# AdalineL/Multi-Modal-GNN

Hardware: AMD Instinct MI355X
Metric: has_lab edges/s, one full training step (new 20 % supervision mask + fwd + weighted-MAE loss + bwd + Adam) of predict_lab_values on the full hetero-graph; message passing over every edge, the two edge heads evaluated on the supervised pairs (the only predictions the loss reads, train.py:366-370) (higher is better)
Workload: dtype f32; 1 GPU; eICU-shape synthetic hetero-graph x100 per GPU, 128-d, 2 SAGE layers x 6 relations, dropout 0.2, supervision mask (20%) redrawn inside every step; patients_per_gpu=183400, has_lab_edges_total=6148400, train_pairs_rank0=4303880, hidden_dim=128, parallelism=single GPU, ranks=1, launch=hipGraph replay

## Files before the change

include/mmgnn.h:

```cpp
#ifndef MMGNN_H
#define MMGNN_H

#include <stddef.h>
#include <stdint.h>

#ifdef __cplusplus
extern "C" {
#endif

#define MMG_OK 0
#define MMG_E_ARG (-1)
#define MMG_E_LAUNCH (-2)
#define MMG_E_WS (-3)

#define MMG_MAX_REL 4

int mmg_version(void);
const char* mmg_last_error(void);

int mmg_stream_create(void** stream_out);
int mmg_stream_destroy(void* stream);

size_t mmg_csr_build_ws_bytes(int64_t n_edges, int64_t n_rows);
int mmg_csr_build(const int64_t* edge_index, int64_t n_edges, int64_t n_rows, int sort_row,
// ... 296 lines not shown
  float drop_p;
  uint64_t seed; uint32_t site; int64_t row_offset; const uint64_t* seed_ptr;
} mmg_small_bn_t;
typedef struct {
  const float* G; const float* Y; float* dY;
  const float* scale; const float* shift; const float* mean; const float* rstd;
  float* dbeta; float* dgamma;
  int64_t M;
  int training;
  int act;
  float drop_p;
  uint64_t seed; uint32_t site; int64_t row_offset; const uint64_t* seed_ptr;
} mmg_small_bn_bwd_t;
int mmg_small_bn_act_group(const mmg_small_bn_t* probs, int n_probs, int N, float momentum, float eps, void* stream);
int mmg_small_bn_bwd_group(const mmg_small_bn_bwd_t* probs, int n_probs, int N, void* stream);

#define MMG_ADAM_MAX_TENSORS 96
#define MMG_SUM_MAX_JOBS 8
int mmg_adam_step(float* p, float* m, float* v, const float* const* grads, const int32_t* offsets, int n_tensors,
                  float lr, float beta1, float beta2, float eps, float weight_decay, float* step, uint32_t* ticket,
                  void* stream);
int mmg_adam_step_dev(float* p, float* m, float* v, const float* const* grads, const int32_t* offsets, int n_tensors,
                      const float* hyper, float* step, uint32_t* ticket, void* stream);
typedef struct {
  float* dst;
  const float* src[4];
  int n_src;
  int len;
  int cols;
  int ld_dst;
  int ld_src[4];
} mmg_sum_job_t;
int mmg_vec_sums(const mmg_sum_job_t* jobs, int n_jobs, void* stream);
#define MMG_COUNTERS_MAX 32
int mmg_counters_add(int64_t* const* counters, const int64_t* incs, int n, void* stream);
int mmg_seed_advance(uint64_t* state , void* stream);
int mmg_fill_zero(void* ptr, size_t bytes, void* stream);

size_t mmg_seg_reduce_ws_bytes(int64_t n, int n_seg);
int mmg_seg_moments(const float* pred, const float* target, const int64_t* seg, int64_t n, int n_seg,
                    double* moments, void* ws, size_t ws_bytes, void* stream);
int mmg_seg_metrics(const float* pred, const float* target, const int64_t* seg, int64_t n, int n_seg,
                    const double* moments, float n_sigma, float* pred_out, double* sums, void* ws, size_t ws_bytes,
                    void* stream);

size_t mmg_knn_impute_ws_bytes(int64_t n_rows, int n_cols, int64_t n_out, int n_neighbors);
int mmg_knn_impute(const float* X, int64_t n_rows, int n_cols, int64_t ld_x, const int32_t* rows, int64_t n_out,
                   int n_neighbors, int weights , float* out, int64_t ld_out, void* ws,
                   size_t ws_bytes, void* stream);

#define MMG_OS_MAX_RANKS 8
size_t mmg_order_stats_ws_bytes(int64_t n);
int mmg_order_stats(const float* a, const float* b, int64_t n, const int64_t* ranks, int n_ranks, float* out,
                    int64_t* nan_count, void* ws, size_t ws_bytes, void* stream);

typedef struct {
  int32_t lo, hi;
  float g;
} mmg_percentile_t;
// ... 124 lines not shown
```

multi-modal-gnn_amd/csrc/optim.hip:

```cpp
#include "common.h"

namespace {

struct AdamTable {
  const float* grad[MMG_ADAM_MAX_TENSORS];
  int32_t off[MMG_ADAM_MAX_TENSORS + 1];
  int n;
};

__global__ __launch_bounds__(256) void k_adam(AdamTable tb, float* __restrict__ p, float* __restrict__ m,
                                              float* __restrict__ v, float lr, float b1, float b2, float eps, float wd,
                                              const float* __restrict__ hyper, const float* __restrict__ step) {
  if (hyper) { lr = hyper[0]; b1 = hyper[1]; b2 = hyper[2]; eps = hyper[3]; wd = hyper[4]; }
  __shared__ float s_bc[3];
  __shared__ int s_off[MMG_ADAM_MAX_TENSORS + 1];
  __shared__ const float* s_grad[MMG_ADAM_MAX_TENSORS];
  for (int i = threadIdx.x; i <= tb.n; i += 256) s_off[i] = tb.off[i];
  for (int i = threadIdx.x; i < tb.n; i += 256) s_grad[i] = tb.grad[i];
  if (threadIdx.x == 0) {
    const float t0 = *step + 1.f;
    s_bc[0] = t0; s_bc[1] = 1.f - powf(b1, t0); s_bc[2] = sqrtf(1.f - powf(b2, t0));
  }
  __syncthreads();
  const float bc1 = s_bc[1], bc2s = s_bc[2];
// ... 40 lines not shown
  const int j = blockIdx.y;
  const int n = jb.len[j], cols = jb.cols[j];
  for (int i = blockIdx.x * 256 + threadIdx.x; i < n; i += gridDim.x * 256) {
    const int r = i / cols, c = i - r * cols;
    float s = jb.src[j][0][(size_t)r * jb.ld_src[j][0] + c];
    for (int q = 1; q < jb.n_src[j]; ++q) s += jb.src[j][q][(size_t)r * jb.ld_src[j][q] + c];
    jb.dst[j][(size_t)r * jb.ld_dst[j] + c] = s;
  }
}

struct CounterTable { int64_t* p[MMG_COUNTERS_MAX]; int64_t inc[MMG_COUNTERS_MAX]; int n; };
__global__ void k_counters_add(CounterTable tb) {
  const int i = threadIdx.x;
  if (i < tb.n) *tb.p[i] += tb.inc[i];
}

__global__ void k_seed_advance(uint64_t* state) {
  uint64_t z = (state[1] += 0x9E3779B97F4A7C15ull);
  z = (z ^ (z >> 30)) * 0xBF58476D1CE4E5B9ull;
  z = (z ^ (z >> 27)) * 0x94D049BB133111EBull;
  state[0] = (z ^ (z >> 31)) >> 2;
}

}

static int adam_launch(float* p, float* m, float* v, const float* const* grads, const int32_t* offsets, int n_tensors,
                       float lr, float beta1, float beta2, float eps, float weight_decay, const float* hyper, float* step,
                       uint32_t* ticket, void* stream) {
  MMG_CHECK_ARG(p && m && v && grads && offsets && step && ticket, "adam_step: null buffer");
  MMG_CHECK_ARG(n_tensors >= 1, "adam_step: no tensors");
  hipStream_t st = (hipStream_t)stream;
  for (int t0 = 0; t0 < n_tensors; t0 += MMG_ADAM_MAX_TENSORS) {
    AdamTable tb;
    const int n = n_tensors - t0 < MMG_ADAM_MAX_TENSORS ? n_tensors - t0 : MMG_ADAM_MAX_TENSORS;
    tb.n = n;
    for (int i = 0; i < n; ++i) { tb.grad[i] = grads[t0 + i]; tb.off[i] = offsets[t0 + i]; }
    tb.off[n] = offsets[t0 + n];
    MMG_CHECK_ARG(tb.off[n] >= tb.off[0], "adam_step: offsets must ascend");
    const int total = tb.off[n] - tb.off[0];
    int nb = (total + 256 * 2 - 1) / (256 * 2);
    if (nb < 1) nb = 1;
    if (nb > 2048) nb = 2048;
    hipLaunchKernelGGL(k_adam, dim3(nb), dim3(256), 0, st, tb, p, m, v, lr, beta1, beta2, eps, weight_decay, hyper, step);
  }
  hipLaunchKernelGGL(k_adam_bump, dim3(1), dim3(1), 0, st, step);
  MMG_CHECK_LAUNCH("adam_step");
  return MMG_OK;
}

extern "C" int mmg_adam_step(float* p, float* m, float* v, const float* const* grads, const int32_t* offsets, int n_tensors,
                             float lr, float beta1, float beta2, float eps, float weight_decay, float* step,
                             uint32_t* ticket, void* stream) {
  return adam_launch(p, m, v, grads, offsets, n_tensors, lr, beta1, beta2, eps, weight_decay, nullptr, step, ticket, stream);
}

extern "C" int mmg_adam_step_dev(float* p, float* m, float* v, const float* const* grads, const int32_t* offsets,
                                 int n_tensors, const float* hyper, float* step, uint32_t* ticket, void* stream) {
  MMG_CHECK_ARG(hyper, "adam_step_dev: null hyper-parameter buffer");
  return adam_launch(p, m, v, grads, offsets, n_tensors, 0.f, 0.f, 0.f, 0.f, 0.f, hyper, step, ticket, stream);
}

extern "C" int mmg_vec_sums(const mmg_sum_job_t* jobs, int n_jobs, void* stream) {
  MMG_CHECK_ARG(jobs && n_jobs >= 1 && n_jobs <= MMG_SUM_MAX_JOBS, "vec_sums: 1..%d jobs", MMG_SUM_MAX_JOBS);
  SumJobs jb;
  jb.n = n_jobs;
  int maxlen = 0;
  for (int j = 0; j < n_jobs; ++j) {
    MMG_CHECK_ARG(jobs[j].dst && jobs[j].n_src >= 1 && jobs[j].n_src <= 4 && jobs[j].len >= 0, "vec_sums: bad job %d", j);
    jb.dst[j] = jobs[j].dst; jb.n_src[j] = jobs[j].n_src; jb.len[j] = jobs[j].len;
    const int cols = jobs[j].cols;
    MMG_CHECK_ARG(cols >= 0 && (cols == 0 || jobs[j].len % cols == 0), "vec_sums: job %d: len is not a multiple of cols", j);
    jb.cols[j] = cols > 0 ? cols : (jobs[j].len > 0 ? jobs[j].len : 1);
    jb.ld_dst[j] = cols > 0 ? jobs[j].ld_dst : 0;
    MMG_CHECK_ARG(cols == 0 || jobs[j].ld_dst >= cols, "vec_sums: job %d: ld_dst < cols", j);
    for (int q = 0; q < 4; ++q) {
      jb.src[j][q] = q < jobs[j].n_src ? jobs[j].src[q] : nullptr;
      jb.ld_src[j][q] = cols > 0 ? jobs[j].ld_src[q] : 0;
      MMG_CHECK_ARG(cols == 0 || q >= jobs[j].n_src || jobs[j].ld_src[q] >= cols, "vec_sums: job %d: ld_src < cols", j);
    }
    for (int q = 0; q < jobs[j].n_src; ++q) MMG_CHECK_ARG(jobs[j].src[q], "vec_sums: job %d has a null source", j);
    if (jobs[j].len > maxlen) maxlen = jobs[j].len;
    for (int i = 0; i < j; ++i) MMG_CHECK_ARG(jobs[i].dst != jobs[j].dst, "vec_sums: jobs %d and %d share a destination", i, j);
// ... 8 lines not shown

extern "C" int mmg_counters_add(int64_t* const* counters, const int64_t* incs, int n, void* stream) {
  MMG_CHECK_ARG(n >= 0 && n <= MMG_COUNTERS_MAX, "counters_add: 0..%d counters", MMG_COUNTERS_MAX);
  if (n == 0) return MMG_OK;
  MMG_CHECK_ARG(counters && incs, "counters_add: null table");
  CounterTable tb;
  tb.n = n;
  for (int i = 0; i < n; ++i) {
    MMG_CHECK_ARG(counters[i], "counters_add: counter %d is null", i);
    tb.p[i] = counters[i]; tb.inc[i] = incs[i];
  }
  hipLaunchKernelGGL(k_counters_add, dim3(1), dim3(64), 0, (hipStream_t)stream, tb);
  MMG_CHECK_LAUNCH("counters_add");
  return MMG_OK;
}

extern "C" int mmg_seed_advance(uint64_t* state, void* stream) {
  MMG_CHECK_ARG(state, "seed_advance: null state");
  hipLaunchKernelGGL(k_seed_advance, dim3(1), dim3(1), 0, (hipStream_t)stream, state);
  MMG_CHECK_LAUNCH("seed_advance");
  return MMG_OK;
}

extern "C" int mmg_fill_zero(void* ptr, size_t bytes, void* stream) {
  if (bytes == 0) return MMG_OK;
  MMG_CHECK_ARG(ptr, "fill_zero: null buffer");
  MMG_CHECK_HIP(mmg_zero_async(ptr, bytes, (hipStream_t)stream), "fill_zero");
  return MMG_OK;
}
```

multi-modal-gnn_amd/model.py:

```python
from __future__ import annotations

import logging
from dataclasses import dataclass, field
from typing import Dict, List, NamedTuple, Optional, Tuple

import torch
import torch.nn as nn
import torch.nn.functional as F

from . import _lib, ops
from .data import GraphPlan, LAB_EDGE, ROW_TYPE, RelCSR, build_plan
from .ops import Pro

EdgeType = Tuple[str, str, str]
SITE_CONV = 16
SITE_H1 = 64
SITE_TYPES_PER_LAYER = 8


def check_dropout_sites(num_layers: int, n_node_types: int):
    if n_node_types > SITE_TYPES_PER_LAYER:
        raise ValueError(f"{n_node_types} node types: the dropout sites of a conv layer hold {SITE_TYPES_PER_LAYER}")
    if SITE_CONV + SITE_TYPES_PER_LAYER * num_layers > SITE_H1:
        raise ValueError(f"num_layers={num_layers}: the dropout sites of the conv layers would run into the pair heads' "
# ... 16 lines not shown

def set_next_bn(sites):
    global NEXT_BN_SITES
    sites = frozenset(sites)
    if not sites <= {"heads", "conv", "enc2", "enc1"}:
        raise ValueError(f"unknown next-BatchNorm site(s): {sorted(sites - {'heads', 'conv', 'enc2', 'enc1'})}")
    NEXT_BN_SITES = sites


FUSED_WGRAD = True


def set_fused_wgrad(on: bool):
    global FUSED_WGRAD
    FUSED_WGRAD = bool(on)


DUAL_ENC = True


def set_dual_enc(on: bool):
    global DUAL_ENC
    DUAL_ENC = bool(on)


FUSED_HEAD_WGRAD = True


def set_fused_head_wgrad(on: bool):
    global FUSED_HEAD_WGRAD
    FUSED_HEAD_WGRAD = bool(on)


def _mangle(et: EdgeType) -> str:
    return "<" + "___".join(et) + ">"


class HeadLists(NamedTuple):
    sel_low: torch.Tensor
    sel_high: torch.Tensor
    counts: torch.Tensor
    n_low: int
    n_high: int
    low_rows: torch.Tensor
    pi_low: torch.Tensor
    deg_low: torch.Tensor
# ... 290 lines not shown
    src: dict
    head: ops.Head
    w1a: torch.Tensor
    w1b: torch.Tensor
    xP: object
    save: Optional[tuple]


class _StepFn(torch.autograd.Function):
    @staticmethod
    def forward(ctx, run, mode, n_out, *params):
        ctx.run = run
        outs = run.run_forward(mode)
        ctx.mark_non_differentiable(*[o for o in outs if not o.is_floating_point()])
        return tuple(outs)

    @staticmethod
    def backward(ctx, *gouts):
        grads = ctx.run.run_backward(gouts)
        return (None, None, None) + tuple(grads)


class _Run:
    def __init__(self, model: HeteroRGCN, data):
        self.m = model
        self.dev = next(model.parameters()).device
        if self.dev.type != "cuda":
            raise ops._lib.MmgError("HeteroRGCN runs on a HIP device only: call model.to('cuda') (no CPU fallback)")
        self.plan: GraphPlan = data if isinstance(data, GraphPlan) else build_plan(data, self.dev)
        self.T = model.training
        self.p = float(model.dropout) if self.T else 0.0
        self.seed_dev = model._seed_dev if self.p > 0 else None
        if self.p > 0 and self.seed_dev is None:
            self.seed = model._dropout_seed if model._dropout_seed is not None else int(
                torch.randint(0, 2 ** 62, (1,)).item())
        else:
            self.seed = 0
        self.comm = model._comm
        self.D = model.hidden_dim
        self.names = [n for n, _ in model.named_parameters()]
        self.params = {n: p for n, p in model.named_parameters()}
        self.grads: Dict[str, torch.Tensor] = {}
        self.partial = set()
        self.tape = {}
        self._nbt = {}
        self.pending = {}
        self.wgrad_jobs = []
        self.static_select = None
        self.forward_select = None
        self.lists_ready = None
        self.pairs = None
        self.lazy_final = False
        ex = getattr(model, "_exec", None) or {}
        mode = ex.get("overlap") or OVERLAP_MODE
        self.next_bn_sites = ex["next_bn"] if ex.get("next_bn") is not None else NEXT_BN_SITES
        self.save_pair_state = ex["save_pair_state"] if ex.get("save_pair_state") is not None else SAVE_PAIR_STATE
        self.fused_wgrad = FUSED_WGRAD
        self.overlap = mode == "on" or (mode == "auto" and self.plan.n_rows >= 16384)
        if self.overlap:
            if getattr(model, "_side_stream", None) is None:
                model._side_stream = torch.cuda.Stream(device=self.dev)
            self.side = model._side_stream
        check_dropout_sites(model.num_layers, len(self.plan.node_types))
        for t in self.plan.node_types:
            if t not in model.embeddings:
                raise KeyError(f"no embedding table for node type '{t}': call model._init_embeddings(data) first")
            if model.embeddings[t].weight.shape[0] != self.plan.num_nodes[t]:
                raise ValueError(f"embedding table for '{t}' has {model.embeddings[t].weight.shape[0]} rows, graph has "
                                 f"{self.plan.num_nodes[t]}")

    def W(self, name) -> torch.Tensor:
        return self.params[name].detach()

    def acc(self, name, g, partial=False):
        if isinstance(name, tuple):
            for n in name:
                self.acc(n, g, partial)
            return
        if name in self.grads:
            if g is not self.grads[name]:
                self.pending.setdefault(name, []).append(g)
        else:
            self.grads[name] = g
        if partial:
            self.partial.add(name)

    def flush_grad_sums(self):
        ops.wgrad_reduce_flush(self.wgrad_jobs)
        levels: List[list] = []
        for name, more in self.pending.items():
            cur, lvl = self.grads[name], 0
            more = [m.reshape(cur.shape) for m in more]
            while more:
                dst = torch.empty_like(cur, memory_format=torch.contiguous_format)
                if len(levels) <= lvl:
                    levels.append([])
                levels[lvl].append((dst, [cur] + more[:3]))
                cur, more, lvl = dst, more[3:], lvl + 1
            self.grads[name] = cur
        self.pending = {}
        for jobs in levels:
            for j0 in range(0, len(jobs), _lib.MMG_SUM_MAX_JOBS):
                ops.vec_sums(jobs[j0:j0 + _lib.MMG_SUM_MAX_JOBS])

    def allreduce(self, t):
        if self.comm is not None:
            self.comm.all_reduce(t)
        return t

    def set_pairs(self, pi, li, pair_ids=None):
        self.pairs = self.m._pairs(pi, li, self.plan.n_rows, pair_ids, self.plan.lab_deg, int(self.m.degree_threshold))
        self.n_pairs = pi.numel()
# ... 11 lines not shown
                pi = torch.arange(P, device=self.dev)
            if pi.device != self.dev:
                raise ops._lib.MmgError("patient_indices must live on the model's device")
            if pi.dtype.is_floating_point or pi.dtype == torch.bool or pi.dim() != 1:
                raise TypeError(f"patient_indices: expected a 1-D integer tensor, got {pi.dtype} {list(pi.shape)}")
            if pi.numel() == 0:
                return torch.empty(0, L, device=self.dev)
            if int(pi.min()) < 0 or int(pi.max()) >= P:
                raise IndexError("patient_indices out of range")
            self.impute_rows = pi.to(torch.int64)
        self.need_grad = need_grad = torch.is_grad_enabled() and any(p.requires_grad for p in self.params.values())
        self.m._last_run = self if need_grad else None
        plist = [self.params[n] for n in self.names]
        if need_grad:
            outs = _StepFn.apply(self, mode, 0, *plist)
        else:
            outs = tuple(self.run_forward(mode))
        if mode in ("predict", "impute"):
            return outs[0]
        return {t: o for t, o in zip(self.out_types, outs)}

    def _bump_counters(self):
        ents = [e for e in self._nbt.values() if e[1]]
        if ents:
            ops.counters_add([b for b, _ in ents], [i for _, i in ents])
        self._nbt = {}

    def run_forward(self, mode):
        outs = self._run_forward(mode)
        self._bump_counters()
        return outs

    def _run_forward(self, mode):
        if mode == "encode":
            enc = self.enc_fwd(0, 1)
            x = self.enc_dict(enc)
            self.tape["mode"] = ("encode", enc)
            self.out_types = list(x.keys())
            return [x[t] if t == ROW_TYPE else x[t].clone() for t in self.out_types]
        if mode == "forward":
            enc = self.enc_fwd(1, 1)
            x, layers = self.layers_fwd(self.enc_dict(enc))
            self.tape["mode"] = ("forward", enc, layers)
            self.out_types = list(x.keys())
            return [x[t] for t in self.out_types]
        self.lazy_final = True
        if mode == "impute":
# ... 742 lines not shown
            ob += tB.numel()
            for t in smalls[w][1:]:
                v.append(flat[o:o + t.numel()].view(t.shape))
                o += t.numel()
            views[w] = v
            tA = heads[w].A
            dA[w] = flat[oa:oa + tA.numel()].view(tA.shape)
            oa += tA.numel()
        gs, join, fused_gp = {}, [], {}
        for which, src, want_low in order:
            hr = rec[which]
            xP, w1a = hr.xP, hr.w1a
            g = ops.Head(dA[which], *views[which])
            sel, n_sel, nb = (bsel_low, bcounts[0:1], ls.n_low) if want_low else (bsel_high, bcounts[1:2], ls.n_high)
            ops.pair_head_bwd(hr.head, g, ls.pi_low if want_low else pi, ps.li, ls.deg_low if want_low else plan.lab_deg, thr,
                              want_low, n_lab, self.p, self.seed, ps.ids, dsrc,
                              self.seed_dev, sel=sel, n_sel=n_sel, n_bound=nb, io_perm=dio, saved=hr.save)
            gs[which] = g
            self.acc(f"{which}.mlp.3.weight", g.W2, partial=True)
            self.acc(f"{which}.mlp.3.bias", g.b2, partial=True)
            self.acc(f"{which}.mlp.6.weight", g.W3.reshape(1, -1), partial=True)
            self.acc(f"{which}.mlp.6.bias", g.b3, partial=True)
            lazy = isinstance(xP, _LazyAct)
            if FUSED_HEAD_WGRAD and ops.linear_dgrad_wgrad_supported(xP.shape[0], D, w1a.shape[0], xP.pro.p if lazy else 0.0):
                fw = ops.FusedWgrad(xP.y, pro=xP.pro) if lazy else ops.FusedWgrad(xP)
                nbn = (ops.NextBN(xP.y, xP.pro, xP.fold)
                       if lazy and not want_low and xP.fold is not None and "heads" in self.next_bn_sites else None)
                fused_gp[which] = ops.linear_dgrad_wgrad(g.A, w1a, fw, next_bn=nbn)
                dW1a = fw.dW
            elif lazy:
                dW1a = ops.linear_wgrad(g.A, xP.y, xP.pro)
            elif xP.shape[0]:
                dW1a = ops.linear_wgrad(g.A, xP)
            else:
                dW1a = ops.zeros(*w1a.shape, device=self.dev)
            dW1b, db1 = ops.linear_wgrad(g.B, src["lab"], with_bias=True)
            dW1 = torch.empty(w1a.shape[0], 2 * D, device=self.dev)
            join += [(dW1[:, :D], [dW1a]), (dW1[:, D:], [dW1b])]
            self.acc(f"{which}.mlp.0.weight", dW1, partial=True)
            self.acc(f"{which}.mlp.0.bias", db1, partial=True)
        ops.vec_sums(join)
        self.allreduce(flat[:n_b])
        for which, src, want_low in order:
            hr, g = rec[which], gs[which]
            xP, w1a, w1b, low_rows = hr.xP, hr.w1a, hr.w1b, ls.low_rows
            glab = ops.linear_fwd(g.B, w1b, w_kn=True)
            if which in fused_gp:
                gP = fused_gp[which]
                if want_low:
                    gsets[which] = {ROW_TYPE: (low_rows, gP), "lab": glab}
                elif isinstance(gP, tuple):
                    gsets[which] = {ROW_TYPE: gP[0], "lab": glab, BN_SUMS: gP[1]}
                else:
                    gsets[which] = {ROW_TYPE: gP, "lab": glab}
            elif want_low:
                if xP.shape[0]:
                    gP = (low_rows, ops.linear_fwd(g.A, w1a, w_kn=True))
                elif self.comm is not None:
                    gP = (low_rows, torch.zeros(0, D, device=self.dev))
                else:
                    gP = None
                gsets[which] = {ROW_TYPE: gP, "lab": glab}
            elif isinstance(xP, _LazyAct) and xP.fold is not None and "heads" in self.next_bn_sites:
                gP, bsums = ops.linear_fwd(g.A, w1a, w_kn=True, next_bn=ops.NextBN(xP.y, xP.pro, xP.fold))
# ... 34 lines not shown
```

multi-modal-gnn_amd/ops.py:

```python
from __future__ import annotations

import ctypes as C
from dataclasses import dataclass
from typing import List, Optional, Sequence

import torch

from . import _lib
from ._lib import (BnFinT, FwdEpiT, HeadGradT, HeadT, NextBnT, PairSavedT, PrologueT, RelT, SmallBnBwdT, SmallBnT, SmallFwdT, SmallWgradT, SumJobT, WgradReduceT, BnBwdT, BnBwdWgradT,
                   check)

BN_MOMENTUM = 0.1
BN_EPS = 1e-5
L2_EPS = 1e-12


def _stream():
    return C.c_void_p(torch.cuda.current_stream().cuda_stream)


def _p(t: Optional[torch.Tensor], dtype=torch.float32, name="tensor", contiguous=True):
    if t is None:
        return None
    where = f"{name}: " if name else ""
# ... 390 lines not shown
        raise ValueError("linear_wgrad: row mismatch")
    if out is None:
        out = torch.empty(N, K, dtype=torch.float32, device=x.device)
        accumulate = False
    dbias = None
    if with_bias:
        dbias = bias_out if (bias_out is not None and accumulate) else torch.empty(N, dtype=torch.float32, device=x.device)
    nb = lib.mmg_linear_wgrad_ws_bytes(M, N, K)
    _tok = _pb("linear_wgrad")
    if defer is None:
        _call("mmg_linear_wgrad", dy, x, _pro(pro), out, dbias, M, N, K, int(accumulate), ws=nb)
    else:
        if accumulate and lib.mmg_linear_wgrad_is_direct(M, N, K) and any(j[2] is out for j in defer):
            wgrad_reduce_flush(defer)
        ws = torch.empty(max(int(nb), 256), dtype=torch.uint8, device=x.device)
        job = WgradReduceT()
        _call("mmg_linear_wgrad_deferred", dy, x, _pro(pro), out, dbias, M, N, K, int(accumulate), C.byref(job), ws=ws)
        defer.append((job, ws, out, dbias))
    _pe(_tok, "linear_wgrad", 4 * (M * N + M * K + N * K), 2 * M * N * K)
    return (out, dbias) if with_bias else out


def wgrad_reduce_flush(jobs: list):
    todo = [j for j in jobs if j[0].slab]
    jobs.clear()
    while todo:
        group, later, seen = [], [], set()
        for j in todo:
            if j[0].dW in seen or len(group) == _lib.MMG_WGRAD_REDUCE_MAX:
                later.append(j)
            else:
                group.append(j)
            seen.add(j[0].dW)
        arr = (WgradReduceT * len(group))(*[j[0] for j in group])
        _call("mmg_wgrad_reduce_group", arr, len(group))
        todo = later


def col_reduce2(a: torch.Tensor, b: Optional[torch.Tensor] = None):
    M, N = a.shape
    out = torch.empty(2, N, dtype=torch.float64, device=a.device)
    _tok = _pb("col_reduce2")
    _call("mmg_col_reduce2", a, b, out, M, N, ws=_lib.load().mmg_col_reduce2_ws_bytes(M, N))
    _pe(_tok, "col_reduce2", 4 * M * N * (2 if b is not None else 1), 0)
    return out


@dataclass
class BNFold:
    scale: torch.Tensor
    shift: torch.Tensor
    mean: torch.Tensor
    rstd: torch.Tensor
    count: int
    training: bool


@dataclass
class NextBN:
# ... 489 lines not shown
        sp = (C.c_void_p * 4)()
        ld = (C.c_int * 4)()
        for q, t in enumerate(srcs):
            if t.numel() != dst.numel():
                raise ValueError("vec_sums: size mismatch")
            sp[q] = _p(t, name="", contiguous=False)
            ld[q] = (views[q + 1][1] or cols) if strided else 0
        arr[j] = SumJobT(_p(dst, name="", contiguous=False), sp, len(srcs), dst.numel(), cols,
                         (views[0][1] or cols) if strided else 0, ld)
    _call("mmg_vec_sums", arr, len(jobs))


def counters_add(counters, incs):
    step = _lib.MMG_COUNTERS_MAX
    for i0 in range(0, len(counters), step):
        cs, ins = counters[i0:i0 + step], incs[i0:i0 + step]
        ptrs = (C.c_void_p * len(cs))(*[_p(c, torch.int64) for c in cs])
        inc = (C.c_int64 * len(cs))(*[int(v) for v in ins])
        _call("mmg_counters_add", ptrs, inc, len(cs))


def seed_advance(state: torch.Tensor):
    _call("mmg_seed_advance", state)


def zeros(*shape, device, dtype=torch.float32):
    t = torch.empty(*shape, device=device, dtype=dtype)
    _call("mmg_fill_zero", _p(t, dtype), t.numel() * t.element_size())
    return t


SMALL_MAX_ROWS = 4096


@dataclass
class SmallFwd:
    x: torch.Tensor
    W: torch.Tensor
    out: Optional[torch.Tensor] = None
    bias: Optional[torch.Tensor] = None
    x2: Optional[torch.Tensor] = None
    W2: Optional[torch.Tensor] = None
    accumulate: bool = False
    w_kn: bool = False


# ... 551 lines not shown
```

multi-modal-gnn_amd/optim.py:

```python
from __future__ import annotations

import ctypes as C
from typing import List

import torch

from . import _lib
from .ops import _call


class Adam(torch.optim.Adam):
    def __init__(self, params, lr=1e-3, betas=(0.9, 0.999), eps=1e-8, weight_decay=0.0):
        self._flat = None
        super().__init__(params, lr=lr, betas=betas, eps=eps, weight_decay=weight_decay)
        self._flat = [self._flatten_group(group) for group in self.param_groups]

    def add_param_group(self, param_group):
        super().add_param_group(param_group)
        if self._flat is not None:
            self._flat.append(self._flatten_group(self.param_groups[-1]))

    def _flatten_group(self, group):
        ps: List[torch.nn.Parameter] = [p for p in group["params"]]
        if not ps:
# ... 23 lines not shown
                  hyper=torch.zeros(5, device=dev), hyper_host=None)
        self._upload_hyper(group, fl)
        return fl

    @staticmethod
    def _hyper_of(group):
        b1, b2 = group["betas"]
        return (float(group["lr"]), float(b1), float(b2), float(group["eps"]), float(group["weight_decay"]))

    def _upload_hyper(self, group, fl):
        h = self._hyper_of(group)
        if h != fl["hyper_host"]:
            if torch.cuda.is_current_stream_capturing():
                raise _lib.MmgError("mmgnn.optim.Adam: hyper-parameters changed inside a stream capture; call sync_hyper() "
                                    "between replays")
            fl["hyper"].copy_(torch.tensor(h, dtype=torch.float32))
            fl["hyper_host"] = h

    def sync_hyper(self):
        for group, fl in zip(self.param_groups, self._flat):
            if fl is not None:
                self._upload_hyper(group, fl)

    @torch.no_grad()
    def step(self, closure=None):
        loss = None
        if closure is not None:
            with torch.enable_grad():
                loss = closure()
        if len(self._flat) != len(self.param_groups):
            raise _lib.MmgError("mmgnn.optim.Adam: param_groups were edited behind add_param_group")
        for group, fl in zip(self.param_groups, self._flat):
            if fl is None:
                continue
            ps = fl["ps"]
            gp = (C.c_void_p * len(ps))()
            for i, p in enumerate(ps):
                g = p.grad
                if g is None:
                    gp[i] = None
                    continue
                if not g.is_cuda or g.dtype != torch.float32 or not g.is_contiguous() or g.numel() != p.numel():
                    raise _lib.MmgError("mmgnn.optim.Adam: gradients must be contiguous fp32 device tensors")
                gp[i] = g.data_ptr()
            self._upload_hyper(group, fl)
            _call("mmg_adam_step_dev", fl["p"], fl["m"], fl["v"], gp, fl["offs"], len(ps), fl["hyper"], fl["step"],
                  fl["ticket"])
        return loss

    def load_state_dict(self, state_dict):
        super().load_state_dict(state_dict)
        with torch.no_grad():
            for fl in self._flat:
                if fl is None:
                    continue
                off = 0
                for p in fl["ps"]:
                    n = p.numel()
                    st = self.state.get(p, {})
                    if "exp_avg" in st:
                        fl["m"][off:off + n].copy_(st["exp_avg"].reshape(-1).to(fl["m"].device))
                        fl["v"][off:off + n].copy_(st["exp_avg_sq"].reshape(-1).to(fl["v"].device))
                        fl["step"].fill_(float(st["step"]))
                    self.state[p] = {"step": fl["step"], "exp_avg": fl["m"][off:off + n].view(p.shape),
                                     "exp_avg_sq": fl["v"][off:off + n].view(p.shape)}
                    off += n
```

multi-modal-gnn_amd/train.py:

```python
from __future__ import annotations

import json
import logging
import time
from pathlib import Path
from typing import Dict, Optional, Tuple

import numpy as np
import torch
import torch.nn as nn
import torch.optim as optim

from .model import build_model, compute_regression_loss

LAB_EDGE = ("patient", "has_lab", "lab")
CAPTURE_ERROR_MODE = "thread_local"


def capture_error_mode() -> str:
    try:
        import torch.distributed as dist
        if dist.is_available() and dist.is_initialized():
            return CAPTURE_ERROR_MODE
    except Exception:
# ... 483 lines not shown
        self._pool = torch.cuda.graph_pool_handle()
        self._begin()
        if self.comm is not None:
            self.comm.on_collective = self._collective
        try:
            body()
        finally:
            if self.comm is not None:
                self.comm.on_collective = None
            self._end()

    def replay(self):
        for kind, x in self.items:
            if kind == "graph":
                x.replay()
            else:
                self.comm.raw_all_reduce(x)

    def release(self):
        self.items = []
        self._cur = None
        self._pool = None
        self.comm = None


class GraphedTrainStep:

    def __init__(self, model, data, pi, li, y, lab_weights, optimizer, sup_mask, loss_fn: str = "mae",
                 n_sup_global: Optional[float] = None, warmup: int = 3):
        self.model, self.data, self.opt = model, data, optimizer
        dev = pi.device
        self.pi, self.li, self.y = pi, li, y
        if loss_fn not in ("mae", "mse", "huber"):
            raise ValueError(f"Unknown loss type: {loss_fn}")
        self.wl = lab_weights[li].contiguous() if loss_fn in ("mae", "mse") else None
        self._sv = _SupervisionState(sup_mask, None, n_sup_global)
        self.sup = self._sv.sup
        self.loss_fn = loss_fn
        model._seed_dev = _new_seed_state(dev)
        self.loss = torch.zeros((), device=dev)
        model.train()
        if len(model.embeddings) == 0:
            model._init_embeddings(data)
        snap = _snapshot_training_state(model, optimizer)
        side = torch.cuda.Stream()
        side.wait_stream(torch.cuda.current_stream())
# ... 101 lines not shown
    def capture_collectives(self) -> bool:
        return self._rec.capture_collectives

    def release(self):
        self._rec.release()
        self._sel_ready = None
        self.comm = None
        self._sv.comm = None

    def _body(self):
        ops, model = self._ops, self.model
        with torch.no_grad():
            for p in self.params:
                p.grad = None
            if self.mask_fraction is not None:
                self._draw_and_select()
            run = self._Run(model, self.plan)
            run.set_pairs(self.pi, self.li, getattr(self.comm, "pair_ids", None) if self.comm else None)
            run.need_grad = True
            run.static_select = self._sel
            run.lists_ready = self._sel_ready
            if self.supervised_heads_only:
                run.forward_select = self._sel
            (pred,) = run.run_forward("predict")
            self.pred = pred
            loss, dpred = ops.pair_loss(pred, self.y, self.wl, self.sup, 1.0, self.loss_fn, self._sv.inv_den,
                                        loss_out=self._loss_out)
            if self.reduce_loss:
                self.comm.all_reduce(loss)
            grads = run.run_backward((dpred,))
            for p, g in zip(self.params, grads):
                if g is not None:
                    p.grad = g
            self.opt.step()
            ops.seed_advance(model._seed_dev)
            self.loss = loss

    def _draw_and_select(self):
        model = self.model
        ids = self._draw_ids
        side = getattr(model, "_side_stream", None)
        if self.comm is not None or side is None:
            self._sv.draw(self.mask_fraction, model._seed_dev, ids, self.n_pairs_global)
            self._select()
            return
        main = torch.cuda.current_stream()
        side.wait_stream(main)
        with torch.cuda.stream(side):
            self._sv.draw(self.mask_fraction, model._seed_dev, ids)
            self._select()
            self._sel_ready = torch.cuda.Event()
            self._sel_ready.record(side)

    def _select(self):
        ops, model = self._ops, self.model
        pairs = model._pairs(self.pi, self.li, self.plan.n_rows,
                             getattr(self.comm, "pair_ids", None) if self.comm else None,
                             self.plan.lab_deg, int(model.degree_threshold))
# ... 76 lines not shown
```

Baseline: 2.831 billion edges/s.

## Fuse weight-grad slab reduction with gradient sums and merge step-counter kernels

Adds a grouped grad-finish kernel that reduces the split-K weight-gradient slabs and folds the pending gradient sums into the same launch, levelled by write/read dependencies. It also merges the Adam step bump, seed advance and batch counters into one tiny kernel at the end of the step. The aim is fewer kernel launches and fewer passes over gradient buffers in the captured graph. In exchange it adds complex host-side dependency and overlap checks, and a risk of ordering bugs between the fused jobs.

```diff
diff --git a/include/mmgnn.h b/include/mmgnn.h
--- a/include/mmgnn.h
+++ b/include/mmgnn.h
@@ -342,6 +342,8 @@
                   void* stream);
 int mmg_adam_step_dev(float* p, float* m, float* v, const float* const* grads, const int32_t* offsets, int n_tensors,
                       const float* hyper, float* step, uint32_t* ticket, void* stream);
+int mmg_adam_update_dev(float* p, float* m, float* v, const float* const* grads, const int32_t* offsets, int n_tensors,
+                        const float* hyper, float* step, void* stream);
 typedef struct {
   float* dst;
   const float* src[4];
@@ -352,9 +354,15 @@
   int ld_src[4];
 } mmg_sum_job_t;
 int mmg_vec_sums(const mmg_sum_job_t* jobs, int n_jobs, void* stream);
+#define MMG_GRAD_FINISH_MAX 24
+#define MMG_GRAD_FINISH_SERIES 4
+int mmg_grad_finish_group(const mmg_wgrad_reduce_t* series, int n_series, const mmg_sum_job_t* sums, int n_sums,
+                          void* stream);
 #define MMG_COUNTERS_MAX 32
 int mmg_counters_add(int64_t* const* counters, const int64_t* incs, int n, void* stream);
 int mmg_seed_advance(uint64_t* state , void* stream);
+int mmg_step_advance(float* adam_step, uint64_t* seed_state, int64_t* const* counters, const int64_t* incs, int n_counters,
+                     void* stream);
 int mmg_fill_zero(void* ptr, size_t bytes, void* stream);
 
 size_t mmg_seg_reduce_ws_bytes(int64_t n, int n_seg);
diff --git a/multi-modal-gnn_amd/csrc/grad_finish.hip b/multi-modal-gnn_amd/csrc/grad_finish.hip
--- /dev/null
+++ b/multi-modal-gnn_amd/csrc/grad_finish.hip
@@ -0,0 +1,210 @@
+#include "common.h"
+#include <vector>
+
+namespace {
+
+struct GfJob {
+  const float* slab[MMG_GRAD_FINISH_SERIES]; int n_split[MMG_GRAD_FINISH_SERIES]; int n_series;
+  int64_t n4;
+  float* dW; float* dbias; int64_t nk4;
+  int accumulate;
+  const float* src[4]; int n_src; int ld_src[4];
+  int cols; int ld_dst;
+};
+struct GradFinishTable { GfJob j[MMG_GRAD_FINISH_MAX]; };
+static_assert(sizeof(GradFinishTable) <= 4096 - 64, "the job table must fit the kernarg segment");
+
+__device__ __forceinline__ size_t gf_offset(int64_t e, int cols, int ld) {
+  if (cols == 0) return (size_t)e;
+  const int64_t r = e / cols;
+  return (size_t)(r * ld + (e - r * cols));
+}
+
+__global__ __launch_bounds__(256) void k_grad_finish_group(GradFinishTable tb) {
+  __shared__ f32x4 part[16][16];
+  const GfJob& jb = tb.j[blockIdx.y];
+  if (jb.n_series == 0) {
+    const int64_t n = jb.n4;
+    for (int64_t i = (int64_t)blockIdx.x * 256 + threadIdx.x; i < n; i += (int64_t)gridDim.x * 256) {
+      float s = jb.src[0][gf_offset(i, jb.cols, jb.ld_src[0])];
+      for (int q = 1; q < jb.n_src; ++q) s += jb.src[q][gf_offset(i, jb.cols, jb.ld_src[q])];
+      jb.dW[gf_offset(i, jb.cols, jb.ld_dst)] = s;
+    }
+    return;
+  }
+  const int e = threadIdx.x & 15, g = threadIdx.x >> 4;
+  const int64_t i4 = (int64_t)blockIdx.x * 16 + e;
+  if ((int64_t)blockIdx.x * 16 >= jb.n4) return;
+  const bool live = i4 < jb.n4, in_w = i4 < jb.nk4;
+  f32x4* o = nullptr;
+  if (g == 0 && live)
+    o = in_w ? reinterpret_cast<f32x4*>(jb.dW + gf_offset(i4 * 4, jb.cols, jb.ld_dst))
+             : reinterpret_cast<f32x4*>(jb.dbias) + (i4 - jb.nk4);
+  f32x4 val = {0.f, 0.f, 0.f, 0.f};
+  for (int s = 0; s < jb.n_series; ++s) {
+    f32x4 acc = {0.f, 0.f, 0.f, 0.f};
+    const int n_split = jb.n_split[s];
+    if (live) {
+      const f32x4* base = reinterpret_cast<const f32x4*>(jb.slab[s]) + i4;
+      int sidx = g;
+      for (; sidx + 7 * 16 < n_split; sidx += 8 * 16) {
+        f32x4 v[8];
+#pragma unroll
+        for (int u = 0; u < 8; ++u) v[u] = base[(size_t)(sidx + u * 16) * jb.n4];
+#pragma unroll
+        for (int u = 0; u < 8; ++u) acc += v[u];
+      }
+      for (; sidx < n_split; sidx += 16) acc += base[(size_t)sidx * jb.n4];
+    }
+    if (s) __syncthreads();
+    part[g][e] = acc;
+    __syncthreads();
+    if (o) {
+      f32x4 t = part[0][e];
+#pragma unroll
+      for (int q = 1; q < 16; ++q) t += part[q][e];
+      if (s == 0) val = jb.accumulate ? (*o + t) : t;
+      else val = val + t;
+    }
+  }
+  if (o) {
+    if (in_w)
+      for (int q = 0; q < jb.n_src; ++q)
+        val = val + *reinterpret_cast<const f32x4*>(jb.src[q] + gf_offset(i4 * 4, jb.cols, jb.ld_src[q]));
+    *o = val;
+  }
+}
+
+struct GfRect { const float* p; int64_t rows, cols, ld; };
+
+static bool gf_overlap(const GfRect& a, const GfRect& b) {
+  if (!a.p || !b.p || a.rows <= 0 || b.rows <= 0 || a.cols <= 0 || b.cols <= 0) return false;
+  const uintptr_t a0 = (uintptr_t)a.p, a1 = (uintptr_t)(a.p + (a.rows - 1) * a.ld + a.cols);
+  const uintptr_t b0 = (uintptr_t)b.p, b1 = (uintptr_t)(b.p + (b.rows - 1) * b.ld + b.cols);
+  if (a1 <= b0 || b1 <= a0) return false;
+  if (a.rows > 1 && b.rows > 1 && a.ld == b.ld && (a0 - b0) % 4 == 0) {
+    const int64_t ld = a.ld;
+    int64_t d = ((int64_t)b0 - (int64_t)a0) / 4 % ld;
+    if (d < 0) d += ld;
+    if (d >= a.cols && d + b.cols <= ld) return false;
+  }
+  return true;
+}
+
+static GfRect gf_rect(const float* p, int64_t n_elem, int cols, int ld) {
+  if (cols > 0) return GfRect{p, n_elem / cols, cols, ld};
+  return GfRect{p, 1, n_elem, n_elem};
+}
+
+}
+
+extern "C" int mmg_grad_finish_group(const mmg_wgrad_reduce_t* series, int n_series, const mmg_sum_job_t* sums, int n_sums,
+                                     void* stream) {
+  const char* what = "grad_finish_group";
+  MMG_CHECK_ARG(n_series >= 0 && n_sums >= 0 && n_series + n_sums >= 1, "%s: no jobs", what);
+  MMG_CHECK_ARG((series || n_series == 0) && (sums || n_sums == 0), "%s: null job list", what);
+  std::vector<GfJob> jobs;
+  std::vector<const float*> unwritten;
+  jobs.reserve((size_t)n_series + n_sums);
+  for (int i = 0; i < n_series; ++i) {
+    const mmg_wgrad_reduce_t& e = series[i];
+    MMG_CHECK_ARG(e.dW, "%s: series %d: null destination", what, i);
+    MMG_CHECK_ARG(e.slab && e.n_split > 0 && (uintptr_t)e.slab % 16 == 0, "%s: series %d: bad slabs", what, i);
+    MMG_CHECK_ARG(e.n4 > 0 && e.n4 < ((int64_t)1 << 40) && e.nk4 >= 0 && e.nk4 <= e.n4, "%s: series %d: bad n4 / nk4", what, i);
+    MMG_CHECK_ARG(e.nk4 == e.n4 || e.dbias, "%s: series %d: a bias tail without dbias", what, i);
+    GfJob* host = nullptr;
+    for (GfJob& b : jobs)
+      if (b.dW == e.dW) host = &b;
+    if (host) {
+      MMG_CHECK_ARG(e.accumulate && host->n4 == e.n4 && host->nk4 == e.nk4 && host->dbias == e.dbias &&
+                        host->n_series < MMG_GRAD_FINISH_SERIES,
+                    "%s: series %d cannot join the job that writes its dW (it belongs in a later launch)", what, i);
+      host->slab[host->n_series] = e.slab; host->n_split[host->n_series] = e.n_split; ++host->n_series;
+      continue;
+    }
+    GfJob b = {};
+    b.slab[0] = e.slab; b.n_split[0] = e.n_split; b.n_series = 1;
+    b.n4 = e.n4; b.dW = e.dW; b.dbias = e.dbias; b.nk4 = e.nk4; b.accumulate = e.accumulate;
+    jobs.push_back(b);
+    unwritten.push_back(nullptr);
+  }
+  const size_t n_slab_jobs = jobs.size();
+  std::vector<const float*> key(n_slab_jobs);
+  std::vector<bool> consumed(n_slab_jobs, false);
+  for (size_t j = 0; j < n_slab_jobs; ++j) key[j] = jobs[j].dW;
+  for (int i = 0; i < n_sums; ++i) {
+    const mmg_sum_job_t& e = sums[i];
+    MMG_CHECK_ARG(e.dst && e.n_src >= 1 && e.n_src <= 4 && e.len >= 0, "%s: sum %d: bad job", what, i);
+    for (int q = 0; q < e.n_src; ++q) MMG_CHECK_ARG(e.src[q], "%s: sum %d has a null source", what, i);
+    MMG_CHECK_ARG(e.cols >= 0 && (e.cols == 0 || (e.len % e.cols == 0 && e.ld_dst >= e.cols)), "%s: sum %d: bad cols / ld_dst", what, i);
+    for (int q = 0; q < e.n_src; ++q) MMG_CHECK_ARG(e.cols == 0 || e.ld_src[q] >= e.cols, "%s: sum %d: ld_src < cols", what, i);
+    size_t h = n_slab_jobs;
+    for (size_t j = 0; j < n_slab_jobs; ++j)
+      if (key[j] == e.src[0]) h = j;
+    if (h < n_slab_jobs && !consumed[h] && (int64_t)e.len == jobs[h].nk4 * 4) {
+      GfJob& b = jobs[h];
+      MMG_CHECK_ARG(!b.accumulate || e.dst == key[h], "%s: sum %d: an accumulating series keeps its dW as the destination", what, i);
+      consumed[h] = true;
+      if (e.dst != key[h]) unwritten[h] = key[h];
+      b.dW = e.dst; b.cols = e.cols; b.ld_dst = e.cols ? e.ld_dst : 0;
+      b.n_src = e.n_src - 1;
+      for (int q = 1; q < e.n_src; ++q) { b.src[q - 1] = e.src[q]; b.ld_src[q - 1] = e.cols ? e.ld_src[q] : 0; }
+      continue;
+    }
+    GfJob b = {};
+    b.n4 = e.len; b.dW = e.dst; b.n_src = e.n_src; b.cols = e.cols; b.ld_dst = e.cols ? e.ld_dst : 0;
+    for (int q = 0; q < e.n_src; ++q) { b.src[q] = e.src[q]; b.ld_src[q] = e.cols ? e.ld_src[q] : 0; }
+    jobs.push_back(b);
+    unwritten.push_back(nullptr);
+  }
+  const int n_jobs = (int)jobs.size();
+  for (int j = 0; j < n_jobs; ++j) {
+    const GfJob& b = jobs[j];
+    if (b.n_series == 0) continue;
+    bool al = (uintptr_t)b.dW % 16 == 0 && (uintptr_t)b.dbias % 16 == 0 && b.cols % 4 == 0 && b.ld_dst % 4 == 0 &&
+              (b.cols == 0 || (b.nk4 * 4) % b.cols == 0);
+    for (int q = 0; q < b.n_src; ++q) al = al && (uintptr_t)b.src[q] % 16 == 0 && b.ld_src[q] % 4 == 0;
+    MMG_CHECK_ARG(al, "%s: job %d: with slabs, addresses, cols and strides are multiples of four elements", what, j);
+  }
+  for (int j = 0; j < n_jobs; ++j) {
+    const GfJob& b = jobs[j];
+    const int64_t nw = b.n_series > 0 ? b.nk4 * 4 : b.n4;
+    const GfRect dw = gf_rect(b.dW, nw, b.cols, b.ld_dst);
+    const GfRect db = b.n_series > 0 && b.nk4 < b.n4 ? GfRect{b.dbias, 1, (b.n4 - b.nk4) * 4, 0} : GfRect{nullptr, 0, 0, 0};
+    const GfRect un = unwritten[j] ? GfRect{unwritten[j], 1, nw, nw} : GfRect{nullptr, 0, 0, 0};
+    MMG_CHECK_ARG(!gf_overlap(dw, db), "%s: job %d: dW and dbias overlap", what, j);
+    for (int i = 0; i < n_jobs; ++i) {
+      if (i == j) continue;
+      const GfJob& a = jobs[i];
+      const int64_t na = a.n_series > 0 ? a.nk4 * 4 : a.n4;
+      if (i < j) {
+        const GfRect aw = gf_rect(a.dW, na, a.cols, a.ld_dst);
+        const GfRect ab = a.n_series > 0 && a.nk4 < a.n4 ? GfRect{a.dbias, 1, (a.n4 - a.nk4) * 4, 0} : GfRect{nullptr, 0, 0, 0};
+        MMG_CHECK_ARG(!gf_overlap(dw, aw) && !gf_overlap(dw, ab) && !gf_overlap(db, aw) && !gf_overlap(db, ab),
+                      "%s: jobs %d and %d write overlapping destinations", what, i, j);
+      }
+      for (int q = 0; q < a.n_src; ++q) {
+        const GfRect sr = gf_rect(a.src[q], na, a.cols, a.ld_src[q]);
+        MMG_CHECK_ARG(!gf_overlap(dw, sr) && !gf_overlap(db, sr) && !gf_overlap(un, sr),
+                      "%s: job %d reads the destination of job %d (it belongs in a later launch)", what, i, j);
+      }
+    }
+  }
+  for (int j0 = 0; j0 < n_jobs; j0 += MMG_GRAD_FINISH_MAX) {
+    GradFinishTable tb;
+    const int n = n_jobs - j0 < MMG_GRAD_FINISH_MAX ? n_jobs - j0 : MMG_GRAD_FINISH_MAX;
+    int64_t nb = 0;
+    for (int j = 0; j < n; ++j) {
+      const GfJob& b = tb.j[j] = jobs[j0 + j];
+      int64_t need = b.n_series > 0 ? (b.n4 + 15) / 16 : (b.n4 + 256 * 4 - 1) / (256 * 4);
+      if (b.n_series == 0 && need > 64) need = 64;
+      if (need > nb) nb = need;
+    }
+    if (nb == 0) continue;
+    MMG_CHECK_ARG(nb <= 0x7FFFFFFF, "%s: too many workgroups", what);
+    MMG_LAUNCH(MMG_PROBE_LINEAR_WGRAD_REDUCE, 0, 0, 0, 0, (k_grad_finish_group), dim3((unsigned)nb, (unsigned)n), dim3(256), 0,
+               (hipStream_t)stream, tb);
+    MMG_CHECK_LAUNCH(what);
+  }
+  return MMG_OK;
+}
diff --git a/multi-modal-gnn_amd/csrc/optim.hip b/multi-modal-gnn_amd/csrc/optim.hip
--- a/multi-modal-gnn_amd/csrc/optim.hip
+++ b/multi-modal-gnn_amd/csrc/optim.hip
@@ -86,11 +86,23 @@
   state[0] = (z ^ (z >> 31)) >> 2;
 }
 
+__global__ void k_step_advance(float* __restrict__ step, uint64_t* __restrict__ seed, CounterTable tb) {
+  const int i = threadIdx.x;
+  if (i < tb.n) *tb.p[i] += tb.inc[i];
+  if (i == 0 && step) *step += 1.f;
+  if (i == 0 && seed) {
+    uint64_t z = (seed[1] += 0x9E3779B97F4A7C15ull);
+    z = (z ^ (z >> 30)) * 0xBF58476D1CE4E5B9ull;
+    z = (z ^ (z >> 27)) * 0x94D049BB133111EBull;
+    seed[0] = (z ^ (z >> 31)) >> 2;
+  }
+}
+
 }
 
 static int adam_launch(float* p, float* m, float* v, const float* const* grads, const int32_t* offsets, int n_tensors,
                        float lr, float beta1, float beta2, float eps, float weight_decay, const float* hyper, float* step,
-                       uint32_t* ticket, void* stream) {
+                       uint32_t* ticket, void* stream, bool bump = true) {
   MMG_CHECK_ARG(p && m && v && grads && offsets && step && ticket, "adam_step: null buffer");
   MMG_CHECK_ARG(n_tensors >= 1, "adam_step: no tensors");
   hipStream_t st = (hipStream_t)stream;
@@ -107,7 +119,7 @@
     if (nb > 2048) nb = 2048;
     hipLaunchKernelGGL(k_adam, dim3(nb), dim3(256), 0, st, tb, p, m, v, lr, beta1, beta2, eps, weight_decay, hyper, step);
   }
-  hipLaunchKernelGGL(k_adam_bump, dim3(1), dim3(1), 0, st, step);
+  if (bump) hipLaunchKernelGGL(k_adam_bump, dim3(1), dim3(1), 0, st, step);
   MMG_CHECK_LAUNCH("adam_step");
   return MMG_OK;
 }
@@ -122,6 +134,13 @@
                                  int n_tensors, const float* hyper, float* step, uint32_t* ticket, void* stream) {
   MMG_CHECK_ARG(hyper, "adam_step_dev: null hyper-parameter buffer");
   return adam_launch(p, m, v, grads, offsets, n_tensors, 0.f, 0.f, 0.f, 0.f, 0.f, hyper, step, ticket, stream);
+}
+
+extern "C" int mmg_adam_update_dev(float* p, float* m, float* v, const float* const* grads, const int32_t* offsets,
+                                   int n_tensors, const float* hyper, float* step, void* stream) {
+  MMG_CHECK_ARG(hyper, "adam_update_dev: null hyper-parameter buffer");
+  uint32_t unused = 0;
+  return adam_launch(p, m, v, grads, offsets, n_tensors, 0.f, 0.f, 0.f, 0.f, 0.f, hyper, step, &unused, stream, false);
 }
 
 extern "C" int mmg_vec_sums(const mmg_sum_job_t* jobs, int n_jobs, void* stream) {
@@ -176,6 +195,22 @@
   return MMG_OK;
 }
 
+extern "C" int mmg_step_advance(float* adam_step, uint64_t* seed_state, int64_t* const* counters, const int64_t* incs,
+                                int n_counters, void* stream) {
+  MMG_CHECK_ARG(n_counters >= 0 && n_counters <= MMG_COUNTERS_MAX, "step_advance: 0..%d counters", MMG_COUNTERS_MAX);
+  MMG_CHECK_ARG(n_counters == 0 || (counters && incs), "step_advance: null table");
+  if (!adam_step && !seed_state && n_counters == 0) return MMG_OK;
+  CounterTable tb;
+  tb.n = n_counters;
+  for (int i = 0; i < n_counters; ++i) {
+    MMG_CHECK_ARG(counters[i], "step_advance: counter %d is null", i);
+    tb.p[i] = counters[i]; tb.inc[i] = incs[i];
+  }
+  hipLaunchKernelGGL(k_step_advance, dim3(1), dim3(64), 0, (hipStream_t)stream, adam_step, seed_state, tb);
+  MMG_CHECK_LAUNCH("step_advance");
+  return MMG_OK;
+}
+
 extern "C" int mmg_fill_zero(void* ptr, size_t bytes, void* stream) {
   if (bytes == 0) return MMG_OK;
   MMG_CHECK_ARG(ptr, "fill_zero: null buffer");
diff --git a/multi-modal-gnn_amd/model.py b/multi-modal-gnn_amd/model.py
--- a/multi-modal-gnn_amd/model.py
+++ b/multi-modal-gnn_amd/model.py
@@ -62,6 +62,14 @@
 def set_dual_enc(on: bool):
     global DUAL_ENC
     DUAL_ENC = bool(on)
+
+
+GRAD_FINISH = True
+
+
+def set_grad_finish(on: bool):
+    global GRAD_FINISH
+    GRAD_FINISH = bool(on)
 
 
 FUSED_HEAD_WGRAD = True
@@ -398,6 +406,9 @@
 
 
 class _Run:
+    grad_finish = False
+    defer_counters = None
+
     def __init__(self, model: HeteroRGCN, data):
         self.m = model
         self.dev = next(model.parameters()).device
@@ -422,6 +433,8 @@
         self._nbt = {}
         self.pending = {}
         self.wgrad_jobs = []
+        self.finish_sums = []
+        self.grad_finish = GRAD_FINISH
         self.static_select = None
         self.forward_select = None
         self.lists_ready = None
@@ -462,8 +475,24 @@
             self.partial.add(name)
 
     def flush_grad_sums(self):
-        ops.wgrad_reduce_flush(self.wgrad_jobs)
         levels: List[list] = []
+        if not self.grad_finish:
+            ops.wgrad_reduce_flush(self.wgrad_jobs)
+        else:
+            first = self.finish_sums
+            self.finish_sums = []
+            outs = {id(e[2]) for e in self.wgrad_jobs if len(e) == 4}
+            for name, more in self.pending.items():
+                cur = self.grads[name]
+                srcs = [cur] + [m.reshape(cur.shape) for m in more[:3]]
+                if id(cur) in outs and sum(1 for g in self.grads.values() if g is cur) == 1:
+                    first.append((cur, srcs))
+                else:
+                    dst = torch.empty_like(cur, memory_format=torch.contiguous_format)
+                    first.append((dst, srcs))
+                    self.grads[name] = dst
+                self.pending[name] = more[3:]
+            ops.grad_finish(self.wgrad_jobs, first)
         for name, more in self.pending.items():
             cur, lvl = self.grads[name], 0
             more = [m.reshape(cur.shape) for m in more]
@@ -521,7 +550,9 @@
 
     def _bump_counters(self):
         ents = [e for e in self._nbt.values() if e[1]]
-        if ents:
+        if self.defer_counters is not None:
+            self.defer_counters += ents
+        elif ents:
             ops.counters_add([b for b, _ in ents], [i for _, i in ents])
         self._nbt = {}
 
@@ -1310,24 +1341,32 @@
             self.acc(f"{which}.mlp.6.weight", g.W3.reshape(1, -1), partial=True)
             self.acc(f"{which}.mlp.6.bias", g.b3, partial=True)
             lazy = isinstance(xP, _LazyAct)
+            hold = [] if self.grad_finish else None
             if FUSED_HEAD_WGRAD and ops.linear_dgrad_wgrad_supported(xP.shape[0], D, w1a.shape[0], xP.pro.p if lazy else 0.0):
-                fw = ops.FusedWgrad(xP.y, pro=xP.pro) if lazy else ops.FusedWgrad(xP)
+                fw = ops.FusedWgrad(xP.y, pro=xP.pro, defer=hold) if lazy else ops.FusedWgrad(xP, defer=hold)
                 nbn = (ops.NextBN(xP.y, xP.pro, xP.fold)
                        if lazy and not want_low and xP.fold is not None and "heads" in self.next_bn_sites else None)
                 fused_gp[which] = ops.linear_dgrad_wgrad(g.A, w1a, fw, next_bn=nbn)
                 dW1a = fw.dW
             elif lazy:
-                dW1a = ops.linear_wgrad(g.A, xP.y, xP.pro)
+                dW1a = ops.linear_wgrad(g.A, xP.y, xP.pro, defer=hold)
             elif xP.shape[0]:
-                dW1a = ops.linear_wgrad(g.A, xP)
+                dW1a = ops.linear_wgrad(g.A, xP, defer=hold)
             else:
                 dW1a = ops.zeros(*w1a.shape, device=self.dev)
             dW1b, db1 = ops.linear_wgrad(g.B, src["lab"], with_bias=True)
             dW1 = torch.empty(w1a.shape[0], 2 * D, device=self.dev)
-            join += [(dW1[:, :D], [dW1a]), (dW1[:, D:], [dW1b])]
+            if hold and hold[0][0].slab:
+                self.wgrad_jobs.append(hold[0] + (dW1[:, :D],))
+                join += [(dW1[:, D:], [dW1b])]
+            else:
+                join += [(dW1[:, :D], [dW1a]), (dW1[:, D:], [dW1b])]
             self.acc(f"{which}.mlp.0.weight", dW1, partial=True)
             self.acc(f"{which}.mlp.0.bias", db1, partial=True)
-        ops.vec_sums(join)
+        if self.grad_finish:
+            self.finish_sums += join
+        else:
+            ops.vec_sums(join)
         self.allreduce(flat[:n_b])
         for which, src, want_low in order:
             hr, g = rec[which], gs[which]
diff --git a/multi-modal-gnn_amd/ops.py b/multi-modal-gnn_amd/ops.py
--- a/multi-modal-gnn_amd/ops.py
+++ b/multi-modal-gnn_amd/ops.py
@@ -436,6 +436,8 @@
 
 
 def wgrad_reduce_flush(jobs: list):
+    if any(len(j) > 4 for j in jobs):
+        return grad_finish(jobs)
     todo = [j for j in jobs if j[0].slab]
     jobs.clear()
     while todo:
@@ -449,6 +451,104 @@
         arr = (WgradReduceT * len(group))(*[j[0] for j in group])
         _call("mmg_wgrad_reduce_group", arr, len(group))
         todo = later
+
+
+def _span(t: torch.Tensor):
+    if t.numel() == 0:
+        return t.data_ptr(), t.data_ptr()
+    last = sum((s - 1) * st for s, st in zip(t.shape, t.stride()))
+    return t.data_ptr(), t.data_ptr() + (last + 1) * t.element_size()
+
+
+def grad_finish(wjobs: list, sums=()):
+    SER = _lib.MMG_GRAD_FINISH_SERIES
+    fjs = []
+    last = {}
+    for ent in wjobs:
+        job = ent[0]
+        if not job.slab:
+            continue
+        view = ent[4] if len(ent) > 4 else None
+        key = view.data_ptr() if view is not None else job.dW
+        prev = last.get(key)
+        if (prev is not None and job.accumulate and len(prev[2]) < SER and prev[5] is None and view is None and not prev[4]
+                and (prev[1][0].n4, prev[1][0].nk4, prev[1][0].dbias) == (job.n4, job.nk4, job.dbias)):
+            prev[2].append((job.slab, job.n_split))
+            continue
+        fj = [key, ent, [(job.slab, job.n_split)], prev[3] + 1 if prev is not None else 0, [], view]
+        fjs.append(fj)
+        last[key] = fj
+    wjobs_keep = list(wjobs)
+    wjobs.clear()
+
+    def writes(fj):
+        ent = fj[1]
+        spans = [_span(fj[5] if fj[5] is not None else ent[2])]
+        if ent[3] is not None:
+            spans.append(_span(ent[3]))
+        return spans
+
+    dense = []
+    for dst, srcs in sums:
+        if not 1 <= len(srcs) <= 4:
+            raise ValueError("grad_finish: 1..4 sources per sum")
+        if any(t.numel() != dst.numel() for t in srcs):
+            raise ValueError("grad_finish: size mismatch")
+        host = None
+        if dst is srcs[0]:
+            host = next((f for f in fjs if f[5] is None and f[1][2] is dst and last[f[0]] is f), None)
+        rest = srcs[1:] if host is not None else srcs
+        lvl, read = 0, [_span(t) for t in rest]
+        for f in fjs:
+            if any(a0 < s1 and s0 < a1 for a0, a1 in writes(f) for s0, s1 in read):
+                lvl = max(lvl, f[3] + 1)
+        ok = (host is not None and lvl <= host[3] and dst.is_contiguous() and dst.numel() == 4 * host[1][0].nk4
+              and all(t.is_contiguous() and t.data_ptr() % 16 == 0 for t in rest))
+        if ok:
+            host[4] = list(rest)
+        else:
+            if host is not None:
+                lvl = max(lvl, host[3] + 1)
+            dense.append((dst, list(srcs), lvl))
+    n_lvl = max([f[3] for f in fjs] + [d[2] for d in dense], default=-1) + 1
+    for lvl in range(n_lvl):
+        group = [f for f in fjs if f[3] == lvl]
+        dgroup = [d for d in dense if d[2] == lvl]
+        series, sjobs = [], []
+        for f in group:
+            job, view = f[1][0], f[5]
+            series.append(job)
+            for slab, n_split in f[2][1:]:
+                series.append(WgradReduceT(slab, job.n4, n_split, job.dW, job.dbias, job.nk4, 1))
+            if view is None and not f[4]:
+                continue
+            sp, ld, cols, ld_dst, dst = (C.c_void_p * 4)(), (C.c_int * 4)(), 0, 0, job.dW
+            if view is not None:
+                if view.dim() != 2 or view.stride(1) != 1 or view.numel() != 4 * job.nk4:
+                    raise ValueError("grad_finish: the destination view must be 2-D with unit column stride and the gradient's size")
+                cols, ld_dst, dst = view.shape[1], view.stride(0), _p(view, name="", contiguous=False)
+            sp[0], ld[0] = job.dW, cols
+            for q, sct in enumerate(f[4], 1):
+                sp[q], ld[q] = _p(sct, name=""), cols
+            sjobs.append(SumJobT(dst, sp, 1 + len(f[4]), 4 * job.nk4, cols, ld_dst, ld))
+        for dst, srcs, _ in dgroup:
+            views = [_rows_view(x) for x in [dst] + srcs]
+            strided = any(c for c, _ in views)
+            cols = 0
+            if strided:
+                if dst.dim() != 2 or any(x.shape != dst.shape for x in srcs):
+                    raise ValueError("grad_finish: strided sums take 2-D tensors of one shape")
+                cols = dst.shape[1]
+            sp, ld = (C.c_void_p * 4)(), (C.c_int * 4)()
+            for q, sct in enumerate(srcs):
+                sp[q] = _p(sct, name="", contiguous=False)
+                ld[q] = (views[q + 1][1] or cols) if strided else 0
+            sjobs.append(SumJobT(_p(dst, name="", contiguous=False), sp, len(srcs), dst.numel(), cols,
+                                 (views[0][1] or cols) if strided else 0, ld))
+        if series or sjobs:
+            _call("mmg_grad_finish_group", (WgradReduceT * max(len(series), 1))(*series), len(series),
+                  (SumJobT * max(len(sjobs), 1))(*sjobs), len(sjobs))
+    del wjobs_keep
 
 
 def col_reduce2(a: torch.Tensor, b: Optional[torch.Tensor] = None):
@@ -984,6 +1084,16 @@
 
 def seed_advance(state: torch.Tensor):
     _call("mmg_seed_advance", state)
+
+
+def step_advance(adam_steps=(), seed_state: Optional[torch.Tensor] = None, counters=(), incs=()):
+    steps, cmax = list(adam_steps), _lib.MMG_COUNTERS_MAX
+    n_calls = max(len(steps), (len(counters) + cmax - 1) // cmax, 1 if seed_state is not None else 0)
+    for i in range(n_calls):
+        cs, ins = counters[i * cmax:(i + 1) * cmax], incs[i * cmax:(i + 1) * cmax]
+        ptrs = (C.c_void_p * max(len(cs), 1))(*[_p(c, torch.int64) for c in cs])
+        inc = (C.c_int64 * max(len(cs), 1))(*[int(v) for v in ins])
+        _call("mmg_step_advance", steps[i] if i < len(steps) else None, seed_state if i == 0 else None, ptrs, inc, len(cs))
 
 
 def zeros(*shape, device, dtype=torch.float32):
diff --git a/multi-modal-gnn_amd/optim.py b/multi-modal-gnn_amd/optim.py
--- a/multi-modal-gnn_amd/optim.py
+++ b/multi-modal-gnn_amd/optim.py
@@ -69,8 +69,11 @@
             if fl is not None:
                 self._upload_hyper(group, fl)
 
+    def step_counters(self):
+        return [fl["step"] for fl in self._flat if fl is not None]
+
     @torch.no_grad()
-    def step(self, closure=None):
+    def step(self, closure=None, bump=True):
         loss = None
         if closure is not None:
             with torch.enable_grad():
@@ -91,8 +94,11 @@
                     raise _lib.MmgError("mmgnn.optim.Adam: gradients must be contiguous fp32 device tensors")
                 gp[i] = g.data_ptr()
             self._upload_hyper(group, fl)
-            _call("mmg_adam_step_dev", fl["p"], fl["m"], fl["v"], gp, fl["offs"], len(ps), fl["hyper"], fl["step"],
-                  fl["ticket"])
+            if bump:
+                _call("mmg_adam_step_dev", fl["p"], fl["m"], fl["v"], gp, fl["offs"], len(ps), fl["hyper"], fl["step"],
+                      fl["ticket"])
+            else:
+                _call("mmg_adam_update_dev", fl["p"], fl["m"], fl["v"], gp, fl["offs"], len(ps), fl["hyper"], fl["step"])
         return loss
 
     def load_state_dict(self, state_dict):
diff --git a/multi-modal-gnn_amd/train.py b/multi-modal-gnn_amd/train.py
--- a/multi-modal-gnn_amd/train.py
+++ b/multi-modal-gnn_amd/train.py
@@ -529,6 +529,14 @@
         self._cur = None
         self._pool = None
         self.comm = None
+
+
+STEP_ADVANCE = True
+
+
+def set_step_advance(on: bool):
+    global STEP_ADVANCE
+    STEP_ADVANCE = bool(on)
 
 
 class GraphedTrainStep:
@@ -676,6 +684,9 @@
             run.lists_ready = self._sel_ready
             if self.supervised_heads_only:
                 run.forward_select = self._sel
+            one = STEP_ADVANCE and hasattr(self.opt, "step_counters")
+            if one:
+                run.defer_counters = []
             (pred,) = run.run_forward("predict")
             self.pred = pred
             loss, dpred = ops.pair_loss(pred, self.y, self.wl, self.sup, 1.0, self.loss_fn, self._sv.inv_den,
@@ -686,8 +697,13 @@
             for p, g in zip(self.params, grads):
                 if g is not None:
                     p.grad = g
-            self.opt.step()
-            ops.seed_advance(model._seed_dev)
+            if one:
+                self.opt.step(bump=False)
+                ents = run.defer_counters
+                ops.step_advance(self.opt.step_counters(), model._seed_dev, [b for b, _ in ents], [i for _, i in ents])
+            else:
+                self.opt.step()
+                ops.seed_advance(model._seed_dev)
             self.loss = loss
 
     def _draw_and_select(self):
```

Result: faster. 2.863 billion edges/s (median of 6 runs) (+1.1%).
